# psweens/VAN-GAN

Measured on AMD Instinct MI355X. Metric: train Mvoxels/s (VanGan.train_step, 128^3 bf16), higher is better.
Workload: dtype bf16; 1 GPU; VanGan.train_step, 128x128x128 volumes, batch 1 per GPU (global 1), clDice on, disc noise+dropout on; parallelism=dp1

## Files before the change

van_gan_amd/csrc/vg_loss.hip:

```cpp
#include "vg_common.h"

static inline int lblocks(int64_t n, int per = 256) { int64_t b = (n + per - 1) / per; return (int)(b > 4095 ? 4095 : (b < 1 ? 1 : b)); }

__device__ __forceinline__ float block_sum(float v, float* sm) {
    v = wave_sum(v);
    const int lane = threadIdx.x & 63, wv = threadIdx.x >> 6;
    __syncthreads();
    if (lane == 0) sm[wv] = v;
    __syncthreads();
    float r = 0.f;
    for (int i = 0; i < (int)(blockDim.x >> 6); ++i) r += sm[i];
    return r;
}

__global__ void mm_init_kernel(float* mm4, int B) {
    const int b = blockIdx.x * blockDim.x + threadIdx.x;
    if (b < B) { mm4[b * 4] = INFINITY; mm4[b * 4 + 1] = -INFINITY; mm4[b * 4 + 2] = 0.f; mm4[b * 4 + 3] = 0.f; }
}
__device__ __forceinline__ void atomic_min_f(float* a, float v) {
    unsigned* ua = (unsigned*)a; unsigned old = *ua;
    while (v < __uint_as_float(old)) { const unsigned prev = atomicCAS(ua, old, __float_as_uint(v)); if (prev == old) break; old = prev; }
}
__device__ __forceinline__ void atomic_max_f(float* a, float v) {
    unsigned* ua = (unsigned*)a; unsigned old = *ua;
// ... 279 lines not shown
    if (!a || !b || !sums3 || n < 1) return VG_EINVAL;
    const int blocks = lblocks(n, 4096) > 255 ? 255 : lblocks(n, 4096);
    hipLaunchKernelGGL(dot_sums_kernel, dim3(blocks), dim3(256), 0, (hipStream_t)stream, a, b, n, sums3);
    return vg_check_launch();
}

__device__ __forceinline__ void gauss3(float* g) {
    const float e = expf(-0.5f * (1.f / 1.5f) * (1.f / 1.5f));
    const float s = 1.f + 2.f * e;
    g[0] = e / s; g[1] = 1.f / s; g[2] = e / s;
}
#define SSIM_C1 1e-4f
#define SSIM_C2 9e-4f
__global__ void ssim_fwd_kernel(const float* t, const float* p, int B, int D, int H, int W, float* acc, float* part) {
    __shared__ float sm[4];
    float g[3]; gauss3(g);
    const int64_t S = (int64_t)D * H * W, total = (int64_t)B * S;
    float loss = 0.f;
    for (int64_t i = (int64_t)blockIdx.x * blockDim.x + threadIdx.x; i < total; i += (int64_t)gridDim.x * blockDim.x) {
        const int w = (int)(i % W); int64_t r = i / W; const int h = (int)(r % H); r /= H; const int d = (int)(r % D); const int b = (int)(r / D);
        float mt = 0.f, mp = 0.f, ett = 0.f, epp = 0.f, etp = 0.f;
        for (int a = -1; a <= 1; ++a) { const int dd = d + a; if (dd < 0 || dd >= D) continue;
            for (int c = -1; c <= 1; ++c) { const int hh = h + c; if (hh < 0 || hh >= H) continue;
                for (int e = -1; e <= 1; ++e) { const int ww = w + e; if (ww < 0 || ww >= W) continue;
                    const float wt = g[a + 1] * g[c + 1] * g[e + 1];
                    const size_t j = (size_t)b * S + ((size_t)dd * H + hh) * W + ww;
                    const float tv = t[j], pv = p[j];
                    mt += wt * tv; mp += wt * pv; ett += wt * tv * tv; epp += wt * pv * pv; etp += wt * tv * pv;
                } } }
        const float stt = ett - mt * mt, spp = epp - mp * mp, stp = etp - mt * mp;
        const float A = 2.f * mt * mp + SSIM_C1, Bq = 2.f * stp + SSIM_C2;
        const float Cq = mt * mt + mp * mp + SSIM_C1, Dq = stt + spp + SSIM_C2;
        const float inv = 1.f / (Cq * Dq);
        const float ssim = A * Bq * inv;
        loss += 1.f - ssim;
        if (part) {
            const float dmu = (2.f * mt * Bq - 2.f * mt * A) * inv - ssim * (2.f * mp * Dq - 2.f * mp * Cq) * inv;
            const float depp = -ssim / Dq;
            const float detp = 2.f * A * inv;
            part[i] = -dmu; part[total + i] = -depp; part[2 * total + i] = -detp;
        }
    }
    loss = block_sum(loss, sm);
    if (threadIdx.x == 0) atomicAdd(acc, loss);
}
extern "C" int vg_ssim_fwd(const float* t, const float* p, int B, int D, int H, int W, float* acc, float* part,
                           vg_stream_t stream) {
    vg_begin();
    if (!t || !p || !acc || B < 1 || D < 1 || H < 1 || W < 1) return VG_EINVAL;
    const int blocks = lblocks((int64_t)B * D * H * W) > 1023 ? 1023 : lblocks((int64_t)B * D * H * W);
    hipLaunchKernelGGL(ssim_fwd_kernel, dim3(blocks), dim3(256), 0, (hipStream_t)stream, t, p, B, D, H, W, acc, part);
    return vg_check_launch();
}
__global__ void ssim_bwd_kernel(const float* t, const float* p, const float* part, int B, int D, int H, int W, float gscale,
                                float* gp, int accum) {
    float g[3]; gauss3(g);
    const int64_t S = (int64_t)D * H * W, total = (int64_t)B * S;
    for (int64_t i = (int64_t)blockIdx.x * blockDim.x + threadIdx.x; i < total; i += (int64_t)gridDim.x * blockDim.x) {
        const int w = (int)(i % W); int64_t r = i / W; const int h = (int)(r % H); r /= H; const int d = (int)(r % D); const int b = (int)(r / D);
        float f0 = 0.f, f1 = 0.f, f2 = 0.f;
        for (int a = -1; a <= 1; ++a) { const int dd = d + a; if (dd < 0 || dd >= D) continue;
            for (int c = -1; c <= 1; ++c) { const int hh = h + c; if (hh < 0 || hh >= H) continue;
                for (int e = -1; e <= 1; ++e) { const int ww = w + e; if (ww < 0 || ww >= W) continue;
                    const float wt = g[a + 1] * g[c + 1] * g[e + 1];
                    const size_t j = (size_t)b * S + ((size_t)dd * H + hh) * W + ww;
                    f0 += wt * part[j]; f1 += wt * part[total + j]; f2 += wt * part[2 * total + j];
                } } }
        const float v = gscale * (f0 + 2.f * p[i] * f1 + t[i] * f2);
        gp[i] = accum ? gp[i] + v : v;
    }
}
extern "C" int vg_ssim_bwd(const float* t, const float* p, const float* part, int B, int D, int H, int W, float gscale,
                           float* gp, int accumulate, vg_stream_t stream) {
    vg_begin();
    if (!t || !p || !part || !gp || B < 1) return VG_EINVAL;
    hipLaunchKernelGGL(ssim_bwd_kernel, dim3(lblocks((int64_t)B * D * H * W)), dim3(256), 0, (hipStream_t)stream, t, p, part, B, D, H, W,
                       gscale, gp, accumulate);
    return vg_check_launch();
}

#define SK_TW 32
#define SK_TH 8
#define SK_TD 8
template <bool ERODE>
__global__ __launch_bounds__(256) void skel_tile_kernel(const float* __restrict__ in, const float* __restrict__ imgj,
                                                        const float* __restrict__ prev, int D, int H, int W, float* __restrict__ out) {
    __shared__ float t[SK_TD + 2][SK_TH + 2][SK_TW + 2];
    const int tid = threadIdx.x;
    const int tiles_w = (W + SK_TW - 1) / SK_TW, tiles_h = (H + SK_TH - 1) / SK_TH;
    int bt = blockIdx.x;
    const int tw = bt % tiles_w; bt /= tiles_w;
    const int th = bt % tiles_h; const int td = bt / tiles_h;
    const int w0 = tw * SK_TW, h0 = th * SK_TH, d0 = td * SK_TD;
    const size_t vol = (size_t)blockIdx.y * D * H * W;
    const float fill = ERODE ? INFINITY : -INFINITY;
    constexpr int NH = (SK_TD + 2) * (SK_TH + 2) * (SK_TW + 2);
    for (int i = tid; i < NH; i += 256) {
        const int x = i % (SK_TW + 2); const int r = i / (SK_TW + 2);
        const int y = r % (SK_TH + 2), z = r / (SK_TH + 2);
        const int gw = w0 + x - 1, gh = h0 + y - 1, gd = d0 + z - 1;
        float v = fill;
        if (gw >= 0 && gw < W && gh >= 0 && gh < H && gd >= 0 && gd < D) v = in[vol + ((size_t)gd * H + gh) * W + gw];
        (&t[0][0][0])[i] = v;
    }
    __syncthreads();
    const int tx = tid & (SK_TW - 1), ty = tid >> 5;
    const int gw = w0 + tx, gh = h0 + ty;
    float p9[3], p5[3];
#pragma unroll
    for (int sl = 0; sl < SK_TD + 2; ++sl) {
        const float a00 = t[sl][ty][tx], a01 = t[sl][ty][tx + 1], a02 = t[sl][ty][tx + 2];
        const float a10 = t[sl][ty + 1][tx], a11 = t[sl][ty + 1][tx + 1], a12 = t[sl][ty + 1][tx + 2];
        const float a20 = t[sl][ty + 2][tx], a21 = t[sl][ty + 2][tx + 1], a22 = t[sl][ty + 2][tx + 2];
        float plus, full;
        if (ERODE) {
            plus = fminf(fminf(fminf(a01, a21), fminf(a10, a12)), a11);
            full = fminf(plus, fminf(fminf(a00, a02), fminf(a20, a22)));
        } else {
            plus = fmaxf(fmaxf(fmaxf(a01, a21), fmaxf(a10, a12)), a11);
            full = fmaxf(plus, fmaxf(fmaxf(a00, a02), fmaxf(a20, a22)));
        }
        p9[sl % 3] = full; p5[sl % 3] = plus;
        if (sl >= 2) {
            const int gd = d0 + sl - 2;
            const int c = (sl - 1) % 3, lo = (sl - 2) % 3, hi = sl % 3;
            const float nb = ERODE ? fminf(p9[c], fminf(p5[lo], p5[hi])) : fmaxf(p9[c], fmaxf(p9[lo], p9[hi]));
            if (gw < W && gh < H && gd < D) {
                const size_t o = vol + ((size_t)gd * H + gh) * W + gw;
                if (ERODE) out[o] = nb;
                else {
                    const float delta = fmaxf(imgj[o] - nb, 0.f);
                    if (prev) { const float sp = prev[o]; out[o] = sp + fmaxf(delta - sp * delta, 0.f); }
                    else out[o] = delta;
                }
            }
        }
    }
}
template <bool AUX>
__global__ __launch_bounds__(256) void skel_chain_kernel(const float* __restrict__ imgs, int64_t n, int iters, int D, int H, int W,
                                                         float* __restrict__ skels, float* __restrict__ deltas, unsigned char* __restrict__ codes) {
    __shared__ float t[SK_TD + 2][SK_TH + 2][SK_TW + 2];
    const int tid = threadIdx.x;
    const int tiles_w = (W + SK_TW - 1) / SK_TW, tiles_h = (H + SK_TH - 1) / SK_TH;
    int bt = blockIdx.x;
    const int tw = bt % tiles_w; bt /= tiles_w;
    const int th = bt % tiles_h; const int td = bt / tiles_h;
    const int w0 = tw * SK_TW, h0 = th * SK_TH, d0 = td * SK_TD;
    const size_t vol = (size_t)blockIdx.y * D * H * W;
    constexpr int NH = (SK_TD + 2) * (SK_TH + 2) * (SK_TW + 2);
    const int tx = tid & (SK_TW - 1), ty = tid >> 5;
    const int gw = w0 + tx, gh = h0 + ty;
    const bool col_ok = gw < W && gh < H;
    float cen[SK_TD], sk[SK_TD];
#pragma unroll
    for (int k = 0; k < SK_TD; ++k) {
        const int gd = d0 + k;
        cen[k] = (col_ok && gd < D) ? imgs[vol + ((size_t)gd * H + gh) * W + gw] : 0.f;
        sk[k] = 0.f;
    }
    for (int j = 0; j <= iters; ++j) {
        const float* __restrict__ in = imgs + (size_t)(j + 1) * n;
        __syncthreads();
        for (int i = tid; i < NH; i += 256) {
            const int x = i % (SK_TW + 2); const int r = i / (SK_TW + 2);
            const int y = r % (SK_TH + 2), z = r / (SK_TH + 2);
            const int qw = w0 + x - 1, qh = h0 + y - 1, qd = d0 + z - 1;
            float v = -INFINITY;
            if (qw >= 0 && qw < W && qh >= 0 && qh < H && qd >= 0 && qd < D) v = in[vol + ((size_t)qd * H + qh) * W + qw];
            (&t[0][0][0])[i] = v;
        }
        __syncthreads();
        float* __restrict__ out = skels + (size_t)j * n;
        float p9[3]; int k9[3];
#pragma unroll
        for (int sl = 0; sl < SK_TD + 2; ++sl) {
            const float a00 = t[sl][ty][tx], a01 = t[sl][ty][tx + 1], a02 = t[sl][ty][tx + 2];
            const float a10 = t[sl][ty + 1][tx], a11 = t[sl][ty + 1][tx + 1], a12 = t[sl][ty + 1][tx + 2];
            const float a20 = t[sl][ty + 2][tx], a21 = t[sl][ty + 2][tx + 1], a22 = t[sl][ty + 2][tx + 2];
            if (AUX) {
                float m = a00; int k = 0;
                if (a01 > m) { m = a01; k = 1; } if (a02 > m) { m = a02; k = 2; }
                if (a10 > m) { m = a10; k = 3; } if (a11 > m) { m = a11; k = 4; } if (a12 > m) { m = a12; k = 5; }
                if (a20 > m) { m = a20; k = 6; } if (a21 > m) { m = a21; k = 7; } if (a22 > m) { m = a22; k = 8; }
                p9[sl % 3] = m; k9[sl % 3] = k;
            } else {
                const float plus = fmaxf(fmaxf(fmaxf(a01, a21), fmaxf(a10, a12)), a11);
                p9[sl % 3] = fmaxf(plus, fmaxf(fmaxf(a00, a02), fmaxf(a20, a22)));
            }
            if (sl >= 2) {
                const int k = sl - 2, gd = d0 + k;
                const float nb = fmaxf(p9[(sl - 1) % 3], fmaxf(p9[(sl - 2) % 3], p9[sl % 3]));
                const float delta = fmaxf(cen[k] - nb, 0.f);
                const float sp = sk[k];
                sk[k] = j ? sp + fmaxf(delta - sp * delta, 0.f) : delta;
                if (col_ok && gd < D) {
                    const size_t o = vol + ((size_t)gd * H + gh) * W + gw;
                    out[o] = sk[k];
                    if (AUX) {
                        float best = p9[(sl - 2) % 3]; int code = k9[(sl - 2) % 3];
                        if (p9[(sl - 1) % 3] > best) { best = p9[(sl - 1) % 3]; code = 9 + k9[(sl - 1) % 3]; }
                        if (p9[sl % 3] > best) { best = p9[sl % 3]; code = 18 + k9[sl % 3]; }
                        deltas[(size_t)j * n + o] = delta; codes[(size_t)j * n + o] = (unsigned char)code;
                    }
                }
            }
        }
#pragma unroll
        for (int k = 0; k < SK_TD; ++k) cen[k] = t[k + 1][ty + 1][tx + 1];
    }
}
__device__ __forceinline__ int64_t sk_off(int code, int H, int W) {
    const int a = code / 9, r = code - a * 9, b = r / 3, c = r - b * 3;
    return ((int64_t)(a - 1) * H + (b - 1)) * W + (c - 1);
}
#define SK_TILE_ORIGIN()                                                                                    \
    const int tiles_w = (W + SK_TW - 1) / SK_TW, tiles_h = (H + SK_TH - 1) / SK_TH;                           \
    int bt_ = blockIdx.x; const int tw_ = bt_ % tiles_w; bt_ /= tiles_w;                                      \
    const int th_ = bt_ % tiles_h, td_ = bt_ / tiles_h;                                                       \
    const int w0 = tw_ * SK_TW, h0 = th_ * SK_TH, d0 = td_ * SK_TD;                                           \
    const size_t vol = (size_t)blockIdx.y * D * H * W;                                                        \
    const int tx = tid & (SK_TW - 1), ty = tid >> 5; const int gw = w0 + tx, gh = h0 + ty;

template <int E>
__device__ __forceinline__ void erode_stage(const float* __restrict__ src, float* __restrict__ dst, int w0, int h0, int d0, int D, int H, int W,
                                            size_t vol, float* __restrict__ out, int tid) {
    constexpr int DD = SK_TD + 2 * E, DH = SK_TH + 2 * E, DW = SK_TW + 2 * E;
    constexpr int SH = DH + 2, SW = DW + 2;
    for (int col = tid; col < DH * DW; col += 256) {
        const int y = col / DW, x = col - y * DW;
        const int gh = h0 - E + y, gw = w0 - E + x;
        const bool col_in = gh >= 0 && gh < H && gw >= 0 && gw < W;
        const bool col_tile = y >= E && y < E + SK_TH && x >= E && x < E + SK_TW;
        float p9[3], p5[3];
#pragma unroll
        for (int sl = 0; sl < DD + 2; ++sl) {
            const float* r0 = src + (sl * SH + y) * SW + x;
            const float* r1 = r0 + SW; const float* r2 = r1 + SW;
            const float a00 = r0[0], a01 = r0[1], a02 = r0[2], a10 = r1[0], a11 = r1[1], a12 = r1[2], a20 = r2[0], a21 = r2[1], a22 = r2[2];
            const float plus = fminf(fminf(fminf(a01, a21), fminf(a10, a12)), a11);
            p9[sl % 3] = fminf(plus, fminf(fminf(a00, a02), fminf(a20, a22))); p5[sl % 3] = plus;
            if (sl >= 2) {
                const int z = sl - 2, gd = d0 - E + z;
                const float nb = fminf(p9[(sl - 1) % 3], fminf(p5[(sl - 2) % 3], p5[sl % 3]));
                const bool in = col_in && gd >= 0 && gd < D;
                if (E > 0) dst[(z * DH + y) * DW + x] = in ? nb : INFINITY;
                if (in && col_tile && z >= E && z < E + SK_TD) out[vol + ((size_t)gd * H + gh) * W + gw] = nb;
            }
        }
    }
}
template <int K>
__global__ __launch_bounds__(256) void erode_multi_kernel(const float* __restrict__ in, int D, int H, int W, int64_t n, float* __restrict__ outs,
                                                          float* __restrict__ copy0) {
    extern __shared__ float sk_lds[];
    constexpr int XD = SK_TD + 2 * K, XH = SK_TH + 2 * K, XW = SK_TW + 2 * K;
    float* A = sk_lds; float* Bf = sk_lds + XD * XH * XW;
    const int tid = threadIdx.x;
    SK_TILE_ORIGIN()
    (void)tx; (void)ty; (void)gw; (void)gh;
    for (int i = tid; i < XD * XH * XW; i += 256) {
        const int x = i % XW; const int r = i / XW; const int y = r % XH, z = r / XH;
        const int qw = w0 - K + x, qh = h0 - K + y, qd = d0 - K + z;
        float v = INFINITY;
        if (qw >= 0 && qw < W && qh >= 0 && qh < H && qd >= 0 && qd < D) {
            const size_t o = vol + ((size_t)qd * H + qh) * W + qw;
            v = in[o];
            if (copy0 && x >= K && x < K + SK_TW && y >= K && y < K + SK_TH && z >= K && z < K + SK_TD) copy0[o] = v;
        }
        A[i] = v;
    }
    __syncthreads();
    erode_stage<K - 1>(A, Bf, w0, h0, d0, D, H, W, vol, outs, tid);
    if constexpr (K >= 2) { __syncthreads(); erode_stage<K - 2>(Bf, A, w0, h0, d0, D, H, W, vol, outs + n, tid); }
    if constexpr (K >= 3) { __syncthreads(); erode_stage<K - 3>(A, Bf, w0, h0, d0, D, H, W, vol, outs + 2 * n, tid); }
    if constexpr (K >= 4) { __syncthreads(); erode_stage<K - 4>(Bf, A, w0, h0, d0, D, H, W, vol, outs + 3 * n, tid); }
}
template <int K>
static void launch_erode_multi(const float* in, int D, int H, int W, int64_t n, float* outs, float* copy0, dim3 grid, hipStream_t s) {
    constexpr int XD = SK_TD + 2 * K, XH = SK_TH + 2 * K, XW = SK_TW + 2 * K;
    constexpr int lds = (XD * XH * XW + (XD - 2) * (XH - 2) * (XW - 2)) * 4;
    static bool attr = false;
    if (!attr) { (void)hipFuncSetAttribute((const void*)erode_multi_kernel<K>, hipFuncAttributeMaxDynamicSharedMemorySize, VG_LDS_LIMIT); attr = true; }
    hipLaunchKernelGGL(erode_multi_kernel<K>, grid, dim3(256), lds, s, in, D, H, W, n, outs, copy0);
}
static dim3 skel_grid(int B, int D, int H, int W) {
    return dim3(((W + SK_TW - 1) / SK_TW) * ((H + SK_TH - 1) / SK_TH) * ((D + SK_TD - 1) / SK_TD), B);
}
__device__ __forceinline__ void sk_load_tile(float (&t)[SK_TD + 2][SK_TH + 2][SK_TW + 2], const float* __restrict__ in, size_t vol,
                                             int w0, int h0, int d0, int D, int H, int W, float fill, int tid) {
    constexpr int NH = (SK_TD + 2) * (SK_TH + 2) * (SK_TW + 2);
    for (int i = tid; i < NH; i += 256) {
        const int x = i % (SK_TW + 2); const int r = i / (SK_TW + 2);
        const int y = r % (SK_TH + 2), z = r / (SK_TH + 2);
        const int gw = w0 + x - 1, gh = h0 + y - 1, gd = d0 + z - 1;
        float v = fill;
        if (gw >= 0 && gw < W && gh >= 0 && gh < H && gd >= 0 && gd < D) v = in[vol + ((size_t)gd * H + gh) * W + gw];
        (&t[0][0][0])[i] = v;
    }
}
__global__ __launch_bounds__(256) void skel_bwd_local_kernel(const float* __restrict__ imgj, const float* __restrict__ imgj1,
                                                             const float* __restrict__ prev, int D, int H, int W,
                                                             float* gs, float* dimgj, float* dimgj1) {
    __shared__ float t[SK_TD + 2][SK_TH + 2][SK_TW + 2];
    const int tid = threadIdx.x;
    SK_TILE_ORIGIN()
    sk_load_tile(t, imgj1, vol, w0, h0, d0, D, H, W, -INFINITY, tid);
    __syncthreads();
    if (gw >= W || gh >= H) return;
    float m9[3]; int k9[3];
#pragma unroll
    for (int sl = 0; sl < SK_TD + 2; ++sl) {
        const float a00 = t[sl][ty][tx], a01 = t[sl][ty][tx + 1], a02 = t[sl][ty][tx + 2];
        const float a10 = t[sl][ty + 1][tx], a11 = t[sl][ty + 1][tx + 1], a12 = t[sl][ty + 1][tx + 2];
        const float a20 = t[sl][ty + 2][tx], a21 = t[sl][ty + 2][tx + 1], a22 = t[sl][ty + 2][tx + 2];
        float m = a00; int k = 0;
        if (a01 > m) { m = a01; k = 1; } if (a02 > m) { m = a02; k = 2; }
        if (a10 > m) { m = a10; k = 3; } if (a11 > m) { m = a11; k = 4; } if (a12 > m) { m = a12; k = 5; }
        if (a20 > m) { m = a20; k = 6; } if (a21 > m) { m = a21; k = 7; } if (a22 > m) { m = a22; k = 8; }
        m9[sl % 3] = m; k9[sl % 3] = k;
        if (sl < 2) continue;
        const int gd = d0 + sl - 2;
        if (gd >= D) continue;
        const size_t i = vol + ((size_t)gd * H + gh) * W + gw;
        float dil = m9[(sl - 2) % 3]; int code = k9[(sl - 2) % 3];
        if (m9[(sl - 1) % 3] > dil) { dil = m9[(sl - 1) % 3]; code = 9 + k9[(sl - 1) % 3]; }
        if (m9[sl % 3] > dil) { dil = m9[sl % 3]; code = 18 + k9[sl % 3]; }
        const float raw = imgj[i] - dil;
        const float delta = fmaxf(raw, 0.f);
        const float g = gs[i];
        float ddelta;
        if (prev) {
            const float sp = prev[i];
            const float u = delta - sp * delta;
            const float dr = u > 0.f ? g : 0.f;
            ddelta = dr * (1.f - sp);
            gs[i] = g - dr * delta;
        } else ddelta = g;
        const float e = raw > 0.f ? ddelta : 0.f;
        if (e != 0.f) { dimgj[i] += e; atomicAdd(&dimgj1[(int64_t)i + sk_off(code, H, W)], -e); }
    }
}
__global__ __launch_bounds__(256) void erode_bwd_kernel(const float* __restrict__ imgj, float* __restrict__ dimgj1,
                                                        int D, int H, int W, float* dimgj) {
    __shared__ float t[SK_TD + 2][SK_TH + 2][SK_TW + 2];
    const int tid = threadIdx.x;
    SK_TILE_ORIGIN()
    sk_load_tile(t, imgj, vol, w0, h0, d0, D, H, W, INFINITY, tid);
    __syncthreads();
    if (gw >= W || gh >= H) return;
    float vC[3], vR[3], vF[3]; int iC[3], iR[3], iF[3];
#pragma unroll
    for (int sl = 0; sl < SK_TD + 2; ++sl) {
        const float a00 = t[sl][ty][tx], a01 = t[sl][ty][tx + 1], a02 = t[sl][ty][tx + 2];
        const float a10 = t[sl][ty + 1][tx], a11 = t[sl][ty + 1][tx + 1], a12 = t[sl][ty + 1][tx + 2];
        const float a20 = t[sl][ty + 2][tx], a21 = t[sl][ty + 2][tx + 1], a22 = t[sl][ty + 2][tx + 2];
        { float m = a01; int k = 0; if (a11 < m) { m = a11; k = 1; } if (a21 < m) { m = a21; k = 2; } vC[sl % 3] = m; iC[sl % 3] = k; }
        { float m = a10; int k = 0; if (a11 < m) { m = a11; k = 1; } if (a12 < m) { m = a12; k = 2; } vR[sl % 3] = m; iR[sl % 3] = k; }
        { float m = a00; int k = 0;
          if (a01 < m) { m = a01; k = 1; } if (a02 < m) { m = a02; k = 2; }
          if (a10 < m) { m = a10; k = 3; } if (a11 < m) { m = a11; k = 4; } if (a12 < m) { m = a12; k = 5; }
          if (a20 < m) { m = a20; k = 6; } if (a21 < m) { m = a21; k = 7; } if (a22 < m) { m = a22; k = 8; }
          vF[sl % 3] = m; iF[sl % 3] = k; }
        if (sl < 2) continue;
        const int gd = d0 + sl - 2;
        if (gd >= D) continue;
        const size_t i = vol + ((size_t)gd * H + gh) * W + gw;
        const float g = dimgj1[i];
        if (g == 0.f) continue;
        dimgj1[i] = 0.f;
        const int lo = (sl - 2) % 3, c = (sl - 1) % 3, hi = sl % 3;
        float best = vC[lo]; int code = iC[lo] * 3 + 1;
        if (vC[c] < best) { best = vC[c]; code = 9 + iC[c] * 3 + 1; }
        if (vC[hi] < best) { best = vC[hi]; code = 18 + iC[hi] * 3 + 1; }
        if (vR[lo] < best) { best = vR[lo]; code = 3 + iR[lo]; }
        if (vR[c] < best) { best = vR[c]; code = 12 + iR[c]; }
        if (vR[hi] < best) { best = vR[hi]; code = 21 + iR[hi]; }
        if (vF[c] < best) { best = vF[c]; code = 9 + iF[c]; }
        atomicAdd(&dimgj[(int64_t)i + sk_off(code, H, W)], g);
    }
}

__global__ __launch_bounds__(256) void skel_erode_code_kernel(const float* __restrict__ in, int D, int H, int W, float* __restrict__ out,
                                                              unsigned char* __restrict__ codes) {
    __shared__ float t[SK_TD + 2][SK_TH + 2][SK_TW + 2];
    const int tid = threadIdx.x;
    SK_TILE_ORIGIN()
    sk_load_tile(t, in, vol, w0, h0, d0, D, H, W, INFINITY, tid);
    __syncthreads();
    float vC[3], vR[3], vF[3]; int iC[3], iR[3], iF[3];
#pragma unroll
    for (int sl = 0; sl < SK_TD + 2; ++sl) {
        const float a00 = t[sl][ty][tx], a01 = t[sl][ty][tx + 1], a02 = t[sl][ty][tx + 2];
        const float a10 = t[sl][ty + 1][tx], a11 = t[sl][ty + 1][tx + 1], a12 = t[sl][ty + 1][tx + 2];
        const float a20 = t[sl][ty + 2][tx], a21 = t[sl][ty + 2][tx + 1], a22 = t[sl][ty + 2][tx + 2];
        { float m = a01; int k = 0; if (a11 < m) { m = a11; k = 1; } if (a21 < m) { m = a21; k = 2; } vC[sl % 3] = m; iC[sl % 3] = k; }
        { float m = a10; int k = 0; if (a11 < m) { m = a11; k = 1; } if (a12 < m) { m = a12; k = 2; } vR[sl % 3] = m; iR[sl % 3] = k; }
        { float m = a00; int k = 0;
          if (a01 < m) { m = a01; k = 1; } if (a02 < m) { m = a02; k = 2; }
          if (a10 < m) { m = a10; k = 3; } if (a11 < m) { m = a11; k = 4; } if (a12 < m) { m = a12; k = 5; }
          if (a20 < m) { m = a20; k = 6; } if (a21 < m) { m = a21; k = 7; } if (a22 < m) { m = a22; k = 8; }
          vF[sl % 3] = m; iF[sl % 3] = k; }
        if (sl >= 2) {
            const int gd = d0 + sl - 2;
            const int lo = (sl - 2) % 3, c = (sl - 1) % 3, hi = sl % 3;
            float best = vC[lo]; int code = iC[lo] * 3 + 1;
            if (vC[c] < best) { best = vC[c]; code = 9 + iC[c] * 3 + 1; }
            if (vC[hi] < best) { best = vC[hi]; code = 18 + iC[hi] * 3 + 1; }
            if (vR[lo] < best) { best = vR[lo]; code = 3 + iR[lo]; }
            if (vR[c] < best) { best = vR[c]; code = 12 + iR[c]; }
            if (vR[hi] < best) { best = vR[hi]; code = 21 + iR[hi]; }
            if (vF[c] < best) { best = vF[c]; code = 9 + iF[c]; }
            if (gw < W && gh < H && gd < D) {
                const size_t o = vol + ((size_t)gd * H + gh) * W + gw;
                out[o] = best; codes[o] = (unsigned char)code;
            }
        }
    }
}

template <int V> __device__ __forceinline__ void sk_ldf(const float* p, int64_t q, float* o) {
    if constexpr (V == 4) { const f32x4 v = ((const f32x4*)p)[q]; o[0] = v[0]; o[1] = v[1]; o[2] = v[2]; o[3] = v[3]; } else o[0] = p[q];
}
template <int V> __device__ __forceinline__ void sk_stf(float* p, int64_t q, const float* o) {
    if constexpr (V == 4) ((f32x4*)p)[q] = (f32x4){o[0], o[1], o[2], o[3]}; else p[q] = o[0];
}
template <int V> __device__ __forceinline__ void sk_ldc(const unsigned char* p, int64_t q, int* o) {
    if constexpr (V == 4) { const unsigned w = ((const unsigned*)p)[q]; o[0] = w & 255; o[1] = (w >> 8) & 255; o[2] = (w >> 16) & 255; o[3] = w >> 24; }
    else o[0] = p[q];
}
template <int V>
__global__ __launch_bounds__(256) void skel_bwd_stream_kernel(const float* __restrict__ d_in, const unsigned char* __restrict__ codeN,
                                                              float* d_acc, float* d_out, int out_accumulate,
                                                              const float* __restrict__ delta, const unsigned char* __restrict__ codeM,
                                                              const float* __restrict__ prev, const float* gs_in, float* gs_out,
                                                              int64_t n, int H, int W) {
    const int64_t nv = n / V;
    for (int64_t q = (int64_t)blockIdx.x * blockDim.x + threadIdx.x; q < nv; q += (int64_t)gridDim.x * blockDim.x) {
        const int64_t i0 = q * V;
        float g_in[V], dl[V], sp[V], g[V]; int cn[V], cm[V];
        if (d_in) { sk_ldf<V>(d_in, q, g_in); sk_ldc<V>(codeN, q, cn); }
        if (delta) { sk_ldf<V>(delta, q, dl); sk_ldf<V>(gs_in, q, g); sk_ldc<V>(codeM, q, cm); if (prev) sk_ldf<V>(prev, q, sp); }
        if (d_in) {
#pragma unroll
            for (int v = 0; v < V; ++v)
                if (g_in[v] != 0.f) atomicAdd(&d_acc[i0 + v + sk_off(cn[v], H, W)], g_in[v]);
        }
        if (delta) {
            float e[V], gn[V];
            bool changed = false;
#pragma unroll
            for (int v = 0; v < V; ++v) {
                float ddelta; gn[v] = g[v];
                if (prev) {
                    const float u = dl[v] - sp[v] * dl[v];
                    const float dr = u > 0.f ? g[v] : 0.f;
                    ddelta = dr * (1.f - sp[v]);
                    gn[v] = g[v] - dr * dl[v];
                } else ddelta = g[v];
                e[v] = dl[v] > 0.f ? ddelta : 0.f;
                changed |= gn[v] != g[v];
                if (e[v] != 0.f) atomicAdd(&d_acc[i0 + v + sk_off(cm[v], H, W)], -e[v]);
            }
            if (prev && (changed || gs_in != gs_out)) sk_stf<V>(gs_out, q, gn);
            if (out_accumulate) {
                float o[V]; sk_ldf<V>(d_out, q, o);
#pragma unroll
                for (int v = 0; v < V; ++v) e[v] += o[v];
            }
            sk_stf<V>(d_out, q, e);
        }
    }
}
extern "C" int vg_soft_skel_fwd(const float* img, int B, int D, int H, int W, int iters, float* imgs, float* skels, void* aux,
                                vg_stream_t stream) {
    vg_begin();
    if (!img || !imgs || !skels || B < 1 || iters < 0) return VG_EINVAL;
    hipStream_t s = (hipStream_t)stream;
    const int64_t n = (int64_t)B * D * H * W;
    const dim3 grid = skel_grid(B, D, H, W);
    const int multi = vg_tune("SKEL_MULTI", 2);
    float* deltas = (float*)aux;
    unsigned char* codeM = aux ? (unsigned char*)(deltas + (size_t)(iters + 1) * n) : nullptr;
    unsigned char* codeN = aux ? codeM + (size_t)(iters + 1) * n : nullptr;
    if (aux) {
        if (hipMemcpyAsync(imgs, img, n * sizeof(float), hipMemcpyDeviceToDevice, s) != hipSuccess) return VG_ELAUNCH;
        for (int j = 0; j <= iters; ++j)
            hipLaunchKernelGGL(skel_erode_code_kernel, grid, dim3(256), 0, s, (const float*)(imgs + j * n), D, H, W, imgs + (j + 1) * n, codeN + (size_t)j * n);
    } else if (multi > 1) {
        for (int j = 0; j <= iters;) {
            const int left = iters + 1 - j;
            const float* in = j ? imgs + j * n : img;
            float* c0 = j ? nullptr : imgs;
            if (left >= 4 && multi >= 4) { launch_erode_multi<4>(in, D, H, W, n, imgs + (j + 1) * n, c0, grid, s); j += 4; }
            else if (left >= 2) { launch_erode_multi<2>(in, D, H, W, n, imgs + (j + 1) * n, c0, grid, s); j += 2; }
            else { launch_erode_multi<1>(in, D, H, W, n, imgs + (j + 1) * n, c0, grid, s); j += 1; }
        }
    } else {
        if (hipMemcpyAsync(imgs, img, n * sizeof(float), hipMemcpyDeviceToDevice, s) != hipSuccess) return VG_ELAUNCH;
        for (int j = 0; j <= iters; ++j)
            hipLaunchKernelGGL(skel_tile_kernel<true>, grid, dim3(256), 0, s, imgs + j * n, (const float*)nullptr, (const float*)nullptr,
                               D, H, W, imgs + (j + 1) * n);
    }
    if (aux) {
        hipLaunchKernelGGL(skel_chain_kernel<true>, grid, dim3(256), 0, s, (const float*)imgs, n, iters, D, H, W, skels, deltas, codeM);
        return vg_check_launch();
    }
    if (vg_tune("SKEL_CHAIN", 1)) {
        hipLaunchKernelGGL(skel_chain_kernel<false>, grid, dim3(256), 0, s, (const float*)imgs, n, iters, D, H, W, skels, (float*)nullptr, (unsigned char*)nullptr);
        return vg_check_launch();
    }
    for (int j = 0; j <= iters; ++j)
        hipLaunchKernelGGL(skel_tile_kernel<false>, grid, dim3(256), 0, s, imgs + (j + 1) * n, imgs + j * n,
                           j ? skels + (j - 1) * n : (const float*)nullptr, D, H, W, skels + j * n);
    return vg_check_launch();
}

extern "C" int vg_soft_skel_bwd(const float* imgs, const float* skels, const float* gskel, int B, int D, int H, int W,
                                int iters, float* work, float* gimg, const void* aux, vg_stream_t stream) {
    vg_begin();
    if (!imgs || !skels || !gskel || !work || !gimg || B < 1 || iters < 0) return VG_EINVAL;
    hipStream_t s = (hipStream_t)stream;
    const int64_t n = (int64_t)B * D * H * W;
    const int blocks = lblocks(n);
    (void)blocks;
    const dim3 grid = skel_grid(B, D, H, W);
    if (aux) {
        const float* deltas = (const float*)aux;
        const unsigned char* codeM = (const unsigned char*)(deltas + (size_t)(iters + 1) * n);
        const unsigned char* codeN = codeM + (size_t)(iters + 1) * n;
        float* gs = work;
        float* d[3] = {work + n, work + 2 * n, work + 3 * n};
        if (hipMemsetAsync(d[(iters + 1) % 3], 0, n * sizeof(float), s) != hipSuccess) return VG_ELAUNCH;
        const bool vec = (n % 4) == 0 && ((((uintptr_t)work | (uintptr_t)gimg | (uintptr_t)gskel | (uintptr_t)skels | (uintptr_t)aux) & 15) == 0);
        const int blocks = lblocks(vec ? n / 4 : n);
        for (int k = iters + 1; k >= 0; --k) {
            const int j = k - 1;
            const bool A = k <= iters, Bp = k >= 1;
            float* d_acc = k == 0 ? gimg : d[k % 3];
            float* d_out = j == 0 ? gimg : (Bp ? d[j % 3] : nullptr);
#define SK_BWD_ARGS A ? (const float*)d[(k + 1) % 3] : (const float*)nullptr, A ? codeN + (size_t)k * n : (const unsigned char*)nullptr, \
                    d_acc, d_out, j == 0 ? 1 : 0, Bp ? deltas + (size_t)j * n : (const float*)nullptr,                                \
                    Bp ? codeM + (size_t)j * n : (const unsigned char*)nullptr,                                                        \
                    (Bp && j > 0) ? skels + (size_t)(j - 1) * n : (const float*)nullptr, k == iters + 1 ? gskel : (const float*)gs, gs, n, H, W
            if (vec) hipLaunchKernelGGL(skel_bwd_stream_kernel<4>, dim3(blocks), dim3(256), 0, s, SK_BWD_ARGS);
            else hipLaunchKernelGGL(skel_bwd_stream_kernel<1>, dim3(blocks), dim3(256), 0, s, SK_BWD_ARGS);
#undef SK_BWD_ARGS
        }
        return vg_check_launch();
    }
    float* gs = work; float* bufA = work + n; float* bufB = work + 2 * n;
    if (hipMemcpyAsync(gs, gskel, n * sizeof(float), hipMemcpyDeviceToDevice, s) != hipSuccess) return VG_ELAUNCH;
    if (hipMemsetAsync(bufA, 0, 2 * n * sizeof(float), s) != hipSuccess) return VG_ELAUNCH;
    for (int j = iters; j >= 0; --j) {
        hipLaunchKernelGGL(skel_bwd_local_kernel, grid, dim3(256), 0, s, imgs + j * n, imgs + (j + 1) * n,
                           j ? skels + (j - 1) * n : (const float*)nullptr, D, H, W, gs, bufB, bufA);
        hipLaunchKernelGGL(erode_bwd_kernel, grid, dim3(256), 0, s, imgs + j * n, bufA, D, H, W, bufB);
        if (j > 0) { float* t = bufA; bufA = bufB; bufB = t; }
    }
    return vg_axpby(bufB, 1.f, nullptr, 0.f, n, gimg, 1, stream);
}

__global__ void cldice_coef_kernel(const float* sums, float w, float alpha, float* coef) {
    if (threadIdx.x != 0 || blockIdx.x != 0) return;
    const float A = sums[0], Bp = sums[1], T = sums[2], Cc = sums[3], Dt = sums[4], P = sums[5], I = sums[6];
    const float pres = (A + 1.f) / (Bp + 1.f), rec = (Cc + 1.f) / (Dt + 1.f);
    const float cl = 1.f - 2.f * pres * rec / (pres + rec);
    const float den = T + P + 1.f;
    const float dice = 1.f - (2.f * I + 1.f) / den;
    const float q = (pres + rec) * (pres + rec);
    const float dcl_dpres = -2.f * rec * rec / q, dcl_drec = -2.f * pres * pres / q;
    coef[0] = w * alpha * dcl_dpres / (Bp + 1.f);
    coef[1] = w * alpha * dcl_dpres * (A + 1.f) / ((Bp + 1.f) * (Bp + 1.f));
    coef[2] = -w * (1.f - alpha) * 2.f / den;
    coef[3] = w * (1.f - alpha) * (2.f * I + 1.f) / (den * den);
    coef[4] = w * alpha * dcl_drec / (Dt + 1.f);
    coef[5] = w * ((1.f - alpha) * dice + alpha * cl);
}
__global__ void cldice_grads_kernel(const float* t, const float* skel_t, const float* coef, int64_t n, float* gskel_p, float* gp, int accum) {
    const float c0 = coef[0], c1 = coef[1], c2 = coef[2], c3 = coef[3], c4 = coef[4];
    for (int64_t i = (int64_t)blockIdx.x * blockDim.x + threadIdx.x; i < n; i += (int64_t)gridDim.x * blockDim.x) {
        const float tv = t[i];
        gskel_p[i] = c0 * tv - c1;
        const float g = c2 * tv + c3 + c4 * skel_t[i];
        gp[i] = accum ? gp[i] + g : g;
    }
}
extern "C" int vg_cldice_coef(const float* sums7, float w, float alpha, float* coef6, vg_stream_t stream) {
    vg_begin();
    if (!sums7 || !coef6) return VG_EINVAL;
    hipLaunchKernelGGL(cldice_coef_kernel, dim3(1), dim3(64), 0, (hipStream_t)stream, sums7, w, alpha, coef6);
    return vg_check_launch();
// ... 99 lines not shown
```

Before: 123.2 Mvoxels/s.

## Vectorize soft-skeleton halo staging with padded LDS rows and batched loads

```diff
diff --git a/van_gan_amd/csrc/vg_loss.hip b/van_gan_amd/csrc/vg_loss.hip
--- a/van_gan_amd/csrc/vg_loss.hip
+++ b/van_gan_amd/csrc/vg_loss.hip
@@ -385,10 +385,115 @@
 #define SK_TW 32
 #define SK_TH 8
 #define SK_TD 8
+#define SK_LP 40
+#define SK_LX 4
+template <int K, int V>
+struct sk_halo {
+    static constexpr int XH = SK_TH + 2 * K, NR = (SK_TD + 2 * K) * XH;
+    static constexpr int PR = SK_TW / V;
+    static constexpr int NI = (NR * PR + 255) / 256, NE = (NR * 2 * K + 255) / 256;
+    static_assert(K >= 1 && K <= SK_LX && NI <= 32 && NE <= 32, "sk_halo: halo does not fit the LDS row / the ok masks");
+    float v[NI][V], e[NE];
+    unsigned oki, oke;
+    static __device__ __forceinline__ bool row_off(int r, int h0, int d0, int D, int H, int W, size_t& off) {
+        const int z = r / XH, y = r - z * XH;
+        const int gd = d0 - K + z, gh = h0 - K + y;
+        off = ((size_t)min(max(gd, 0), D - 1) * H + min(max(gh, 0), H - 1)) * W;
+        return gd >= 0 && gd < D && gh >= 0 && gh < H;
+    }
+    static __device__ __forceinline__ int edge_dx(int c) { return c < K ? c - K : SK_TW - K + c; }
+    __device__ __forceinline__ void issue(const float* __restrict__ in, size_t vol, int w0, int h0, int d0, int D, int H, int W, int tid,
+                                          int k0 = 0, int k1 = NI + NE) {
+        if (k0 == 0) oki = oke = 0u;
+#pragma unroll
+        for (int k = 0; k < NI; ++k) {
+            if (k < k0 || k >= k1) continue;
+            const int i = tid + 256 * k, gw = w0 + (i % PR) * V;
+            size_t off;
+            const bool ok = row_off(i / PR, h0, d0, D, H, W, off) && gw < W;
+            const float* p = in + vol + off + min(gw, W - V);
+            if constexpr (V == 4) { const f32x4 q = *(const f32x4*)p; v[k][0] = q[0]; v[k][1] = q[1]; v[k][2] = q[2]; v[k][3] = q[3]; }
+            else v[k][0] = *p;
+            oki |= (ok ? 1u : 0u) << k;
+        }
+#pragma unroll
+        for (int k = 0; k < NE; ++k) {
+            if (NI + k < k0 || NI + k >= k1) continue;
+            const int i = tid + 256 * k, gw = w0 + edge_dx(i % (2 * K));
+            size_t off;
+            const bool ok = row_off(i / (2 * K), h0, d0, D, H, W, off) && gw >= 0 && gw < W;
+            e[k] = in[vol + off + min(max(gw, 0), W - 1)];
+            oke |= (ok ? 1u : 0u) << k;
+        }
+        __builtin_amdgcn_sched_barrier(0);
+    }
+    __device__ __forceinline__ void commit(float* __restrict__ t, float fill, int tid, int k0 = 0, int k1 = NI + NE) const {
+        float* const s0 = t + (tid / PR) * SK_LP + SK_LX + (tid % PR) * V;
+        float f0[V];
+#pragma unroll
+        for (int c = 0; c < V; ++c) f0[c] = (oki & 1u) ? v[0][c] : fill;
+#pragma unroll
+        for (int k = 0; k < NI; ++k) {
+            const int i = tid + 256 * k, r = i / PR;
+            const bool live = 256 * (k + 1) <= NR * PR || r < NR;
+            if (k < k0 || k >= k1 || (k0 != 0 && !live)) continue;
+            float* d = live ? t + r * SK_LP + SK_LX + (i % PR) * V : s0;
+            const bool ok = (oki >> k) & 1u;
+            float f[V];
+#pragma unroll
+            for (int c = 0; c < V; ++c) f[c] = live ? (ok ? v[k][c] : fill) : f0[c];
+            if constexpr (V == 4) *(f32x4*)d = (f32x4){f[0], f[1], f[2], f[3]};
+            else *d = f[0];
+        }
+#pragma unroll
+        for (int k = 0; k < NE; ++k) {
+            const int i = tid + 256 * k, r = i / (2 * K);
+            const bool live = 256 * (k + 1) <= NR * 2 * K || r < NR;
+            if (NI + k < k0 || NI + k >= k1 || (k0 != 0 && !live)) continue;
+            float* d = live ? t + r * SK_LP + SK_LX + edge_dx(i % (2 * K)) : s0;
+            *d = live ? (((oke >> k) & 1u) ? e[k] : fill) : f0[0];
+        }
+    }
+    __device__ __forceinline__ void file_tile(float* __restrict__ out, size_t vol, int w0, int h0, int d0, int D, int H, int W, int tid,
+                                              int k0, int k1) const {
+#pragma unroll
+        for (int k = 0; k < NI; ++k) {
+            const int i = tid + 256 * k, r = i / PR, z = r / XH, y = r - z * XH;
+            if (k < k0 || k >= k1 || !((oki >> k) & 1u) || z < K || z >= K + SK_TD || y < K || y >= K + SK_TH) continue;
+            float* d = out + vol + ((size_t)(d0 - K + z) * H + (h0 - K + y)) * W + w0 + (i % PR) * V;
+            if constexpr (V == 4) *(f32x4*)d = (f32x4){v[k][0], v[k][1], v[k][2], v[k][3]};
+            else *d = v[k][0];
+        }
+    }
+};
+__host__ __device__ __forceinline__ bool sk_vec_ok(const void* p, const void* q, int W) { return (W & 3) == 0 && ((((uintptr_t)p) | ((uintptr_t)q)) & 15) == 0; }
+#define SK_BATCH 8
+template <int K, int V>
+__device__ __forceinline__ void sk_stage_v(float* __restrict__ t, const float* __restrict__ in, size_t vol, int w0, int h0, int d0, int D, int H,
+                                           int W, float fill, int tid, float* __restrict__ copy0) {
+    sk_halo<K, V> h;
+    constexpr int N = h.NI + h.NE, NB = V == 4 ? N : SK_BATCH;
+#pragma unroll
+    for (int k0 = 0; k0 < N; k0 += NB) {
+        h.issue(in, vol, w0, h0, d0, D, H, W, tid, k0, k0 + NB);
+        h.commit(t, fill, tid, k0, k0 + NB);
+        if (copy0) h.file_tile(copy0, vol, w0, h0, d0, D, H, W, tid, k0, k0 + NB);
+    }
+}
+template <int K>
+__device__ __forceinline__ void sk_stage(float* __restrict__ t, const float* __restrict__ in, size_t vol, int w0, int h0, int d0, int D, int H, int W,
+                                         float fill, int tid, float* __restrict__ copy0 = nullptr) {
+    if (sk_vec_ok(in, copy0, W)) sk_stage_v<K, 4>(t, in, vol, w0, h0, d0, D, H, W, fill, tid, copy0);
+    else sk_stage_v<K, 1>(t, in, vol, w0, h0, d0, D, H, W, fill, tid, copy0);
+}
+#define SK_WIN9(t, sl)                                                                                                              \
+    const float a00 = t[sl][ty][tx + SK_LX - 1], a01 = t[sl][ty][tx + SK_LX], a02 = t[sl][ty][tx + SK_LX + 1];                      \
+    const float a10 = t[sl][ty + 1][tx + SK_LX - 1], a11 = t[sl][ty + 1][tx + SK_LX], a12 = t[sl][ty + 1][tx + SK_LX + 1];          \
+    const float a20 = t[sl][ty + 2][tx + SK_LX - 1], a21 = t[sl][ty + 2][tx + SK_LX], a22 = t[sl][ty + 2][tx + SK_LX + 1];
 template <bool ERODE>
 __global__ __launch_bounds__(256) void skel_tile_kernel(const float* __restrict__ in, const float* __restrict__ imgj,
                                                         const float* __restrict__ prev, int D, int H, int W, float* __restrict__ out) {
-    __shared__ float t[SK_TD + 2][SK_TH + 2][SK_TW + 2];
+    __shared__ __attribute__((aligned(16))) float t[SK_TD + 2][SK_TH + 2][SK_LP];
     const int tid = threadIdx.x;
     const int tiles_w = (W + SK_TW - 1) / SK_TW, tiles_h = (H + SK_TH - 1) / SK_TH;
     int bt = blockIdx.x;
@@ -396,25 +501,14 @@
     const int th = bt % tiles_h; const int td = bt / tiles_h;
     const int w0 = tw * SK_TW, h0 = th * SK_TH, d0 = td * SK_TD;
     const size_t vol = (size_t)blockIdx.y * D * H * W;
-    const float fill = ERODE ? INFINITY : -INFINITY;
-    constexpr int NH = (SK_TD + 2) * (SK_TH + 2) * (SK_TW + 2);
-    for (int i = tid; i < NH; i += 256) {
-        const int x = i % (SK_TW + 2); const int r = i / (SK_TW + 2);
-        const int y = r % (SK_TH + 2), z = r / (SK_TH + 2);
-        const int gw = w0 + x - 1, gh = h0 + y - 1, gd = d0 + z - 1;
-        float v = fill;
-        if (gw >= 0 && gw < W && gh >= 0 && gh < H && gd >= 0 && gd < D) v = in[vol + ((size_t)gd * H + gh) * W + gw];
-        (&t[0][0][0])[i] = v;
-    }
+    sk_stage<1>(&t[0][0][0], in, vol, w0, h0, d0, D, H, W, ERODE ? INFINITY : -INFINITY, tid);
     __syncthreads();
     const int tx = tid & (SK_TW - 1), ty = tid >> 5;
     const int gw = w0 + tx, gh = h0 + ty;
     float p9[3], p5[3];
 #pragma unroll
     for (int sl = 0; sl < SK_TD + 2; ++sl) {
-        const float a00 = t[sl][ty][tx], a01 = t[sl][ty][tx + 1], a02 = t[sl][ty][tx + 2];
-        const float a10 = t[sl][ty + 1][tx], a11 = t[sl][ty + 1][tx + 1], a12 = t[sl][ty + 1][tx + 2];
-        const float a20 = t[sl][ty + 2][tx], a21 = t[sl][ty + 2][tx + 1], a22 = t[sl][ty + 2][tx + 2];
+        SK_WIN9(t, sl)
         float plus, full;
         if (ERODE) {
             plus = fminf(fminf(fminf(a01, a21), fminf(a10, a12)), a11);
@@ -440,10 +534,10 @@
         }
     }
 }
-template <bool AUX>
+template <bool AUX, int V>
 __global__ __launch_bounds__(256) void skel_chain_kernel(const float* __restrict__ imgs, int64_t n, int iters, int D, int H, int W,
                                                          float* __restrict__ skels, float* __restrict__ deltas, unsigned char* __restrict__ codes) {
-    __shared__ float t[SK_TD + 2][SK_TH + 2][SK_TW + 2];
+    __shared__ __attribute__((aligned(16))) float t[SK_TD + 2][SK_TH + 2][SK_LP];
     const int tid = threadIdx.x;
     const int tiles_w = (W + SK_TW - 1) / SK_TW, tiles_h = (H + SK_TH - 1) / SK_TH;
     int bt = blockIdx.x;
@@ -451,7 +545,6 @@
     const int th = bt % tiles_h; const int td = bt / tiles_h;
     const int w0 = tw * SK_TW, h0 = th * SK_TH, d0 = td * SK_TD;
     const size_t vol = (size_t)blockIdx.y * D * H * W;
-    constexpr int NH = (SK_TD + 2) * (SK_TH + 2) * (SK_TW + 2);
     const int tx = tid & (SK_TW - 1), ty = tid >> 5;
     const int gw = w0 + tx, gh = h0 + ty;
     const bool col_ok = gw < W && gh < H;
@@ -459,28 +552,18 @@
 #pragma unroll
     for (int k = 0; k < SK_TD; ++k) {
         const int gd = d0 + k;
-        cen[k] = (col_ok && gd < D) ? imgs[vol + ((size_t)gd * H + gh) * W + gw] : 0.f;
+        cen[k] = imgs[vol + ((size_t)min(gd, D - 1) * H + min(gh, H - 1)) * W + min(gw, W - 1)];
         sk[k] = 0.f;
     }
     for (int j = 0; j <= iters; ++j) {
-        const float* __restrict__ in = imgs + (size_t)(j + 1) * n;
         __syncthreads();
-        for (int i = tid; i < NH; i += 256) {
-            const int x = i % (SK_TW + 2); const int r = i / (SK_TW + 2);
-            const int y = r % (SK_TH + 2), z = r / (SK_TH + 2);
-            const int qw = w0 + x - 1, qh = h0 + y - 1, qd = d0 + z - 1;
-            float v = -INFINITY;
-            if (qw >= 0 && qw < W && qh >= 0 && qh < H && qd >= 0 && qd < D) v = in[vol + ((size_t)qd * H + qh) * W + qw];
-            (&t[0][0][0])[i] = v;
-        }
+        sk_stage_v<1, V>(&t[0][0][0], imgs + (size_t)(j + 1) * n, vol, w0, h0, d0, D, H, W, -INFINITY, tid, nullptr);
         __syncthreads();
         float* __restrict__ out = skels + (size_t)j * n;
         float p9[3]; int k9[3];
 #pragma unroll
         for (int sl = 0; sl < SK_TD + 2; ++sl) {
-            const float a00 = t[sl][ty][tx], a01 = t[sl][ty][tx + 1], a02 = t[sl][ty][tx + 2];
-            const float a10 = t[sl][ty + 1][tx], a11 = t[sl][ty + 1][tx + 1], a12 = t[sl][ty + 1][tx + 2];
-            const float a20 = t[sl][ty + 2][tx], a21 = t[sl][ty + 2][tx + 1], a22 = t[sl][ty + 2][tx + 2];
+            SK_WIN9(t, sl)
             if (AUX) {
                 float m = a00; int k = 0;
                 if (a01 > m) { m = a01; k = 1; } if (a02 > m) { m = a02; k = 2; }
@@ -510,7 +593,7 @@
             }
         }
 #pragma unroll
-        for (int k = 0; k < SK_TD; ++k) cen[k] = t[k + 1][ty + 1][tx + 1];
+        for (int k = 0; k < SK_TD; ++k) cen[k] = t[k + 1][ty + 1][tx + SK_LX];
     }
 }
 __device__ __forceinline__ int64_t sk_off(int code, int H, int W) {
@@ -525,11 +608,11 @@
     const size_t vol = (size_t)blockIdx.y * D * H * W;                                                        \
     const int tx = tid & (SK_TW - 1), ty = tid >> 5; const int gw = w0 + tx, gh = h0 + ty;
 
-template <int E>
+template <int E, int SW>
 __device__ __forceinline__ void erode_stage(const float* __restrict__ src, float* __restrict__ dst, int w0, int h0, int d0, int D, int H, int W,
                                             size_t vol, float* __restrict__ out, int tid) {
     constexpr int DD = SK_TD + 2 * E, DH = SK_TH + 2 * E, DW = SK_TW + 2 * E;
-    constexpr int SH = DH + 2, SW = DW + 2;
+    constexpr int SH = DH + 2;
     for (int col = tid; col < DH * DW; col += 256) {
         const int y = col / DW, x = col - y * DW;
         const int gh = h0 - E + y, gw = w0 - E + x;
@@ -556,33 +639,23 @@
 template <int K>
 __global__ __launch_bounds__(256) void erode_multi_kernel(const float* __restrict__ in, int D, int H, int W, int64_t n, float* __restrict__ outs,
                                                           float* __restrict__ copy0) {
-    extern __shared__ float sk_lds[];
+    extern __shared__ __attribute__((aligned(16))) float sk_lds[];
     constexpr int XD = SK_TD + 2 * K, XH = SK_TH + 2 * K, XW = SK_TW + 2 * K;
-    float* A = sk_lds; float* Bf = sk_lds + XD * XH * XW;
+    float* A = sk_lds; float* Bf = sk_lds + XD * XH * SK_LP;
     const int tid = threadIdx.x;
     SK_TILE_ORIGIN()
     (void)tx; (void)ty; (void)gw; (void)gh;
-    for (int i = tid; i < XD * XH * XW; i += 256) {
-        const int x = i % XW; const int r = i / XW; const int y = r % XH, z = r / XH;
-        const int qw = w0 - K + x, qh = h0 - K + y, qd = d0 - K + z;
-        float v = INFINITY;
-        if (qw >= 0 && qw < W && qh >= 0 && qh < H && qd >= 0 && qd < D) {
-            const size_t o = vol + ((size_t)qd * H + qh) * W + qw;
-            v = in[o];
-            if (copy0 && x >= K && x < K + SK_TW && y >= K && y < K + SK_TH && z >= K && z < K + SK_TD) copy0[o] = v;
-        }
-        A[i] = v;
-    }
+    sk_stage<K>(A, in, vol, w0, h0, d0, D, H, W, INFINITY, tid, copy0);
     __syncthreads();
-    erode_stage<K - 1>(A, Bf, w0, h0, d0, D, H, W, vol, outs, tid);
-    if constexpr (K >= 2) { __syncthreads(); erode_stage<K - 2>(Bf, A, w0, h0, d0, D, H, W, vol, outs + n, tid); }
-    if constexpr (K >= 3) { __syncthreads(); erode_stage<K - 3>(A, Bf, w0, h0, d0, D, H, W, vol, outs + 2 * n, tid); }
-    if constexpr (K >= 4) { __syncthreads(); erode_stage<K - 4>(Bf, A, w0, h0, d0, D, H, W, vol, outs + 3 * n, tid); }
+    erode_stage<K - 1, SK_LP>(A + (SK_LX - K), Bf, w0, h0, d0, D, H, W, vol, outs, tid);
+    if constexpr (K >= 2) { __syncthreads(); erode_stage<K - 2, XW - 2>(Bf, A, w0, h0, d0, D, H, W, vol, outs + n, tid); }
+    if constexpr (K >= 3) { __syncthreads(); erode_stage<K - 3, XW - 4>(A, Bf, w0, h0, d0, D, H, W, vol, outs + 2 * n, tid); }
+    if constexpr (K >= 4) { __syncthreads(); erode_stage<K - 4, XW - 6>(Bf, A, w0, h0, d0, D, H, W, vol, outs + 3 * n, tid); }
 }
 template <int K>
 static void launch_erode_multi(const float* in, int D, int H, int W, int64_t n, float* outs, float* copy0, dim3 grid, hipStream_t s) {
     constexpr int XD = SK_TD + 2 * K, XH = SK_TH + 2 * K, XW = SK_TW + 2 * K;
-    constexpr int lds = (XD * XH * XW + (XD - 2) * (XH - 2) * (XW - 2)) * 4;
+    constexpr int lds = (XD * XH * SK_LP + (XD - 2) * (XH - 2) * (XW - 2)) * 4;
     static bool attr = false;
     if (!attr) { (void)hipFuncSetAttribute((const void*)erode_multi_kernel<K>, hipFuncAttributeMaxDynamicSharedMemorySize, VG_LDS_LIMIT); attr = true; }
     hipLaunchKernelGGL(erode_multi_kernel<K>, grid, dim3(256), lds, s, in, D, H, W, n, outs, copy0);
@@ -590,33 +663,25 @@
 static dim3 skel_grid(int B, int D, int H, int W) {
     return dim3(((W + SK_TW - 1) / SK_TW) * ((H + SK_TH - 1) / SK_TH) * ((D + SK_TD - 1) / SK_TD), B);
 }
-__device__ __forceinline__ void sk_load_tile(float (&t)[SK_TD + 2][SK_TH + 2][SK_TW + 2], const float* __restrict__ in, size_t vol,
-                                             int w0, int h0, int d0, int D, int H, int W, float fill, int tid) {
-    constexpr int NH = (SK_TD + 2) * (SK_TH + 2) * (SK_TW + 2);
-    for (int i = tid; i < NH; i += 256) {
-        const int x = i % (SK_TW + 2); const int r = i / (SK_TW + 2);
-        const int y = r % (SK_TH + 2), z = r / (SK_TH + 2);
-        const int gw = w0 + x - 1, gh = h0 + y - 1, gd = d0 + z - 1;
-        float v = fill;
-        if (gw >= 0 && gw < W && gh >= 0 && gh < H && gd >= 0 && gd < D) v = in[vol + ((size_t)gd * H + gh) * W + gw];
-        (&t[0][0][0])[i] = v;
-    }
-}
 __global__ __launch_bounds__(256) void skel_bwd_local_kernel(const float* __restrict__ imgj, const float* __restrict__ imgj1,
                                                              const float* __restrict__ prev, int D, int H, int W,
                                                              float* gs, float* dimgj, float* dimgj1) {
-    __shared__ float t[SK_TD + 2][SK_TH + 2][SK_TW + 2];
+    __shared__ __attribute__((aligned(16))) float t[SK_TD + 2][SK_TH + 2][SK_LP];
     const int tid = threadIdx.x;
     SK_TILE_ORIGIN()
-    sk_load_tile(t, imgj1, vol, w0, h0, d0, D, H, W, -INFINITY, tid);
+    float o_img[SK_TD], o_gs[SK_TD], o_prev[SK_TD];
+#pragma unroll
+    for (int k = 0; k < SK_TD; ++k) {
+        const size_t i = vol + ((size_t)min(d0 + k, D - 1) * H + min(gh, H - 1)) * W + min(gw, W - 1);
+        o_img[k] = imgj[i]; o_gs[k] = gs[i]; o_prev[k] = prev ? prev[i] : 0.f;
+    }
+    sk_stage<1>(&t[0][0][0], imgj1, vol, w0, h0, d0, D, H, W, -INFINITY, tid);
     __syncthreads();
     if (gw >= W || gh >= H) return;
     float m9[3]; int k9[3];
 #pragma unroll
     for (int sl = 0; sl < SK_TD + 2; ++sl) {
-        const float a00 = t[sl][ty][tx], a01 = t[sl][ty][tx + 1], a02 = t[sl][ty][tx + 2];
-        const float a10 = t[sl][ty + 1][tx], a11 = t[sl][ty + 1][tx + 1], a12 = t[sl][ty + 1][tx + 2];
-        const float a20 = t[sl][ty + 2][tx], a21 = t[sl][ty + 2][tx + 1], a22 = t[sl][ty + 2][tx + 2];
+        SK_WIN9(t, sl)
         float m = a00; int k = 0;
         if (a01 > m) { m = a01; k = 1; } if (a02 > m) { m = a02; k = 2; }
         if (a10 > m) { m = a10; k = 3; } if (a11 > m) { m = a11; k = 4; } if (a12 > m) { m = a12; k = 5; }
@@ -629,12 +694,11 @@
         float dil = m9[(sl - 2) % 3]; int code = k9[(sl - 2) % 3];
         if (m9[(sl - 1) % 3] > dil) { dil = m9[(sl - 1) % 3]; code = 9 + k9[(sl - 1) % 3]; }
         if (m9[sl % 3] > dil) { dil = m9[sl % 3]; code = 18 + k9[sl % 3]; }
-        const float raw = imgj[i] - dil;
+        const float raw = o_img[sl - 2] - dil, g = o_gs[sl - 2];
         const float delta = fmaxf(raw, 0.f);
-        const float g = gs[i];
         float ddelta;
         if (prev) {
-            const float sp = prev[i];
+            const float sp = o_prev[sl - 2];
             const float u = delta - sp * delta;
             const float dr = u > 0.f ? g : 0.f;
             ddelta = dr * (1.f - sp);
@@ -646,18 +710,16 @@
 }
 __global__ __launch_bounds__(256) void erode_bwd_kernel(const float* __restrict__ imgj, float* __restrict__ dimgj1,
                                                         int D, int H, int W, float* dimgj) {
-    __shared__ float t[SK_TD + 2][SK_TH + 2][SK_TW + 2];
+    __shared__ __attribute__((aligned(16))) float t[SK_TD + 2][SK_TH + 2][SK_LP];
     const int tid = threadIdx.x;
     SK_TILE_ORIGIN()
-    sk_load_tile(t, imgj, vol, w0, h0, d0, D, H, W, INFINITY, tid);
+    sk_stage<1>(&t[0][0][0], imgj, vol, w0, h0, d0, D, H, W, INFINITY, tid);
     __syncthreads();
     if (gw >= W || gh >= H) return;
     float vC[3], vR[3], vF[3]; int iC[3], iR[3], iF[3];
 #pragma unroll
     for (int sl = 0; sl < SK_TD + 2; ++sl) {
-        const float a00 = t[sl][ty][tx], a01 = t[sl][ty][tx + 1], a02 = t[sl][ty][tx + 2];
-        const float a10 = t[sl][ty + 1][tx], a11 = t[sl][ty + 1][tx + 1], a12 = t[sl][ty + 1][tx + 2];
-        const float a20 = t[sl][ty + 2][tx], a21 = t[sl][ty + 2][tx + 1], a22 = t[sl][ty + 2][tx + 2];
+        SK_WIN9(t, sl)
         { float m = a01; int k = 0; if (a11 < m) { m = a11; k = 1; } if (a21 < m) { m = a21; k = 2; } vC[sl % 3] = m; iC[sl % 3] = k; }
         { float m = a10; int k = 0; if (a11 < m) { m = a11; k = 1; } if (a12 < m) { m = a12; k = 2; } vR[sl % 3] = m; iR[sl % 3] = k; }
         { float m = a00; int k = 0;
@@ -686,17 +748,15 @@
 
 __global__ __launch_bounds__(256) void skel_erode_code_kernel(const float* __restrict__ in, int D, int H, int W, float* __restrict__ out,
                                                               unsigned char* __restrict__ codes) {
-    __shared__ float t[SK_TD + 2][SK_TH + 2][SK_TW + 2];
+    __shared__ __attribute__((aligned(16))) float t[SK_TD + 2][SK_TH + 2][SK_LP];
     const int tid = threadIdx.x;
     SK_TILE_ORIGIN()
-    sk_load_tile(t, in, vol, w0, h0, d0, D, H, W, INFINITY, tid);
+    sk_stage<1>(&t[0][0][0], in, vol, w0, h0, d0, D, H, W, INFINITY, tid);
     __syncthreads();
     float vC[3], vR[3], vF[3]; int iC[3], iR[3], iF[3];
 #pragma unroll
     for (int sl = 0; sl < SK_TD + 2; ++sl) {
-        const float a00 = t[sl][ty][tx], a01 = t[sl][ty][tx + 1], a02 = t[sl][ty][tx + 2];
-        const float a10 = t[sl][ty + 1][tx], a11 = t[sl][ty + 1][tx + 1], a12 = t[sl][ty + 1][tx + 2];
-        const float a20 = t[sl][ty + 2][tx], a21 = t[sl][ty + 2][tx + 1], a22 = t[sl][ty + 2][tx + 2];
+        SK_WIN9(t, sl)
         { float m = a01; int k = 0; if (a11 < m) { m = a11; k = 1; } if (a21 < m) { m = a21; k = 2; } vC[sl % 3] = m; iC[sl % 3] = k; }
         { float m = a10; int k = 0; if (a11 < m) { m = a11; k = 1; } if (a12 < m) { m = a12; k = 2; } vR[sl % 3] = m; iR[sl % 3] = k; }
         { float m = a00; int k = 0;
@@ -806,11 +866,13 @@
                                D, H, W, imgs + (j + 1) * n);
     }
     if (aux) {
-        hipLaunchKernelGGL(skel_chain_kernel<true>, grid, dim3(256), 0, s, (const float*)imgs, n, iters, D, H, W, skels, deltas, codeM);
+        if (sk_vec_ok(imgs, nullptr, W)) hipLaunchKernelGGL((skel_chain_kernel<true, 4>), grid, dim3(256), 0, s, (const float*)imgs, n, iters, D, H, W, skels, deltas, codeM);
+        else hipLaunchKernelGGL((skel_chain_kernel<true, 1>), grid, dim3(256), 0, s, (const float*)imgs, n, iters, D, H, W, skels, deltas, codeM);
         return vg_check_launch();
     }
     if (vg_tune("SKEL_CHAIN", 1)) {
-        hipLaunchKernelGGL(skel_chain_kernel<false>, grid, dim3(256), 0, s, (const float*)imgs, n, iters, D, H, W, skels, (float*)nullptr, (unsigned char*)nullptr);
+        if (sk_vec_ok(imgs, nullptr, W)) hipLaunchKernelGGL((skel_chain_kernel<false, 4>), grid, dim3(256), 0, s, (const float*)imgs, n, iters, D, H, W, skels, (float*)nullptr, (unsigned char*)nullptr);
+        else hipLaunchKernelGGL((skel_chain_kernel<false, 1>), grid, dim3(256), 0, s, (const float*)imgs, n, iters, D, H, W, skels, (float*)nullptr, (unsigned char*)nullptr);
         return vg_check_launch();
     }
     for (int j = 0; j <= iters; ++j)
```

Result: no change. 123.0 Mvoxels/s (-0.1%).
